# TencentAI4S/HuDiff

Measured on AMD Instinct MI355X. Metric: humanized sequences/sec (full T-step sample) on HuAb348, higher is better.
Workload: dtype f32-equivalent: fp16 hi+lo split, 3 MFMA / product, f32 accumulate; pruned tail + static branch f32

## Files before the change

hudiff_amd/csrc/hd_api.hip:

```cpp
#include "../../include/hudiff_hip.h"
#include "hd_kernels.hip.h"
#include "hd_tail_fused.hip.h"
#include "hd_attn_fused.hip.h"
#include "hd_chain.hip.h"

#include <cmath>
#include <cstdarg>
#include <cstdio>
#include <cstdlib>
#include <cstring>
#include <map>
#include <string>
#include <vector>

using namespace hd;

static thread_local std::string g_err;
static thread_local std::string g_launch_err;

static HdStatus fail(HdStatus st, const char* fmt, ...) {
    char buf[1024];
    va_list ap;
    va_start(ap, fmt);
    vsnprintf(buf, sizeof(buf), fmt, ap);
// ... 69 lines not shown
    {HD_OPT_BIG_MIN_ROWS, "HUDIFF_BIG_ROWS", 8192, 1, OPT_BIG, {}, 0, false},
    {HD_OPT_LNSYNC_LEVEL, "HUDIFF_X3_LNSYNC", 2, 0, 2, {}, 0, false},
    {HD_OPT_TAIL_FORM, "HUDIFF_TAIL", 2, 0, 2, {0, 2}, 2, false},
    {HD_OPT_TAIL_MAX_ROWS, "HUDIFF_TAIL_MAX_B", 64, 0, OPT_BIG, {}, 0, false},
    {HD_OPT_SMALL_GRID, "HUDIFF_X3_SMALL_GRID", 320, 0, OPT_BIG, {}, 0, false},
    {HD_OPT_TINY_GRID, "HUDIFF_X3_TINY_GRID", 150, 0, OPT_BIG, {}, 0, false},
    {HD_OPT_LOADER_WAVES, "HUDIFF_X3_LOADERS", 1, 0, 1, {}, 0, false},
    {HD_OPT_TINY_STAGES, "HUDIFF_X3_TINY_NS", 3, 2, 3, {}, 0, false},
    {HD_OPT_SMALL_STAGES, "HUDIFF_X3_SMALL_NS", 0, 0, 3, {0, 2, 3}, 3, false},
    {HD_OPT_SMALL_STAGES3_MAX_GRID, "HUDIFF_X3_SMALL_NS3_MAX", 256, 0, OPT_BIG, {}, 0, false},
    {HD_OPT_ATTN_QSPLIT_MAX_GRID, "HUDIFF_ATTN_QSPLIT_MAX", 128, 0, OPT_BIG, {}, 0, false},
    {HD_OPT_ATTN_WAVES, "HUDIFF_ATTN_WAVES", 12, 8, 12, {8, 12}, 2, false},
    {HD_OPT_LOOP_GRAPH, "HUDIFF_LOOP_GRAPH", 0, 0, 1, {}, 0, false},
    {HD_OPT_PRUNE_VALUE_VIA_ROWS, "HUDIFF_PRUNE_V", 1, 0, 1, {}, 0, false},
    {HD_OPT_SPLIT_TILE, "HUDIFF_X3_TILE", 0, 0, 512, {0, 128, 256, 512}, 4, false},
    {HD_OPT_GEMM_SMALL_TILES, "HUDIFF_GEMM_SMALL", 1536, 0, OPT_BIG, {}, 0, false},
    {HD_OPT_STORE_NT, "HUDIFF_ST_NT", 0, 0, 1, {}, 0, false},
    {HD_OPT_SPLIT_LAYER_MASK, "HUDIFF_X3_MASK", 3, 0, 3, {}, 0, true},
    {HD_OPT_SPLIT_ATTN, "HUDIFF_X3_ATTN", 1, 0, 1, {}, 0, false},
    {HD_OPT_FUSED_ATTN, "HUDIFF_FUSED_ATTN", 1, 0, 1, {}, 0, false},
    {HD_OPT_FUSED_ATTN_MIN_GRID, "HUDIFF_FUSED_ATTN_MIN_GRID", 128, 0, OPT_BIG, {}, 0, false},
    {HD_OPT_BN_CHAIN, "HUDIFF_BN_CHAIN", 0, 0, 3, {}, 0, true},
    {HD_OPT_BN_CHAIN_MIN_TILES, "HUDIFF_BN_CHAIN_MIN_TILES", 128, 0, OPT_BIG, {}, 0, false},
};
static bool opt_legal(const OptDef& d, int64_t v) {
    if (v < d.lo || v > d.hi) return false;
    if (d.nset == 0) return true;
    for (int i = 0; i < d.nset; ++i) if (d.set[i] == v) return true;
    return false;
}

struct HdModel {
    HdConfig cfg{};
    int device = 0;
    hipStream_t stream = nullptr;
    bool finalized = false;
    std::map<std::string, HostTensor> host;
    int nseg = 1, d = 0, dh = 0, D = 0, Dh = 0, A = 0, Fd = 0, L = 0;
    float p_enc = 0.f, p_conv = 0.f;
    float* blob = nullptr;
    uint16_t* blobx = nullptr;
    int precision_req = HD_PRECISION_DEFAULT, precision = HD_PRECISION_SPLIT;
    int64_t opt[HD_OPT_COUNT] = {};
    bool debug_lnsync_scatter = false;
    bool x3 = false;
    bool x3_suspended = false;
    int64_t range_fallbacks = 0;
    bool attn_x3 = true;
    int lnsync_level_cfg = 2, lnsync_level = 2;
    int64_t lnsync_fallbacks = 0;
    bool last_call_repeated = false;
    bool lnsync_cross_xcd = false;
    const float* emb = nullptr;
    std::vector<ByteNetW> enc, conv;
    std::vector<AttBlockW> att;
    RegionW regw{};
    SideW sidew{};
    const float *pos_w1 = nullptr, *pos_b1 = nullptr, *pos_w2 = nullptr, *pos_b2 = nullptr;
    HeadW head{};
    const float *rope_cos = nullptr, *rope_sin = nullptr, *rope_cs = nullptr;
    float* side_vec = nullptr;
    float2* emb_stats = nullptr;
    float* qnoise = nullptr; size_t qnoise_cap = 0;
    struct Lane {
        hipStream_t stream = nullptr;
        RunState* rs = nullptr;
        Workspace ws;
// ... 83 lines not shown
    if (c.kind != HD_KIND_ANTIBODY && c.kind != HD_KIND_NANOBODY) return fail(HD_ERR_INVALID, "hd_create: kind %d", c.kind);
    if (c.att_model != c.nhead * ATT_HD)
        return fail(HD_ERR_UNSUPPORTED, "hd_create: head dim %d/%d unsupported (kernels implement 64)", c.att_model, c.nhead);
    const int nkt = (c.max_len + 15) / 16;
    if (nkt != 19 && nkt != 10)
        return fail(HD_ERR_UNSUPPORTED, "hd_create: max_len %d unsupported (291 or 152)", c.max_len);
    if (c.d_model % 8 || c.sum_d_model % 8 || c.dim_feedforward % 4 || c.d_model > 512 || c.sum_d_model > 1024)
        return fail(HD_ERR_UNSUPPORTED, "hd_create: widths must be multiples of 8 (d_model<=512, sum_d_model<=1024)");
    if (c.r_embedding > 8 || c.s_embedding > 8 || c.n_tokens < 23 || c.n_tokens > 64)
        return fail(HD_ERR_UNSUPPORTED, "hd_create: r_embedding/s_embedding <= 8, n_tokens in [23,64]");
    if (c.kind == HD_KIND_ANTIBODY) {
        if (c.h_len <= 0 || c.h_len >= c.max_len) return fail(HD_ERR_INVALID, "hd_create: h_len %d", c.h_len);
        if (c.sum_d_model != 3 * c.d_model) return fail(HD_ERR_INVALID, "hd_create: sum_d_model != 3*d_model");
    } else {
        if (c.h_len != c.max_len) return fail(HD_ERR_INVALID, "hd_create: nanobody h_len must equal max_len");
        if (c.sum_d_model != 2 * c.d_model) return fail(HD_ERR_INVALID, "hd_create: sum_d_model != 2*d_model");
    }
    if (c.kernel_size != 7 && c.kernel_size != 5 && c.kernel_size != 3)
        return fail(HD_ERR_UNSUPPORTED, "hd_create: kernel_size %d", c.kernel_size);
    if (!(c.dropout >= 0.f && c.dropout < 1.f)) return fail(HD_ERR_INVALID, "hd_create: dropout %f", c.dropout);
    for (int a : {c.enc_act, c.conv_act})
        if (a != HD_ACT_RELU && a != HD_ACT_GELU) return fail(HD_ERR_INVALID, "hd_create: activation %d", a);

    int ndev = hd_device_count();
    if (ndev <= 0) return fail(HD_ERR_NO_DEVICE, "hd_create: no HIP device visible (this library has no CPU path)");
    if (device < 0 || device >= ndev) return fail(HD_ERR_INVALID, "hd_create: device %d out of range [0,%d)", device, ndev);
    HIP_TRY(hipSetDevice(device));
    hipDeviceProp_t prop;
    HIP_TRY(hipGetDeviceProperties(&prop, device));
    if (strncmp(prop.gcnArchName, "gfx950", 6) != 0)
        return fail(HD_ERR_NO_DEVICE, "hd_create: device %d is %s, kernels are built for gfx950 only", device, prop.gcnArchName);
    HdModel* m = new HdModel();
    m->cfg = c;
    for (const OptDef& d : OPTS) {
        m->opt[d.id] = d.def;
        if (const char* e = getenv(d.env)) {
            const int64_t v = atoll(e);
            if (opt_legal(d, v)) m->opt[d.id] = v;
            else {
                if (d.nset == 0) m->opt[d.id] = v < d.lo ? d.lo : d.hi;
                if (!getenv("HUDIFF_QUIET"))
                    fprintf(stderr, "[hudiff_hip] %s=%s is not a legal value of that option: %s %lld\n", d.env, e,
                            d.nset == 0 ? "clamped to" : "ignored, the default stays", (long long)m->opt[d.id]);
            }
        }
    }
    if (!getenv("HUDIFF_QUIET")) {
        static const char* const removed[] = {"HUDIFF_GEMM_NBUF", "HUDIFF_PFF3_APPLY", "HUDIFF_ENC_FUSED", "HUDIFF_ENC_ABL", "HUDIFF_X3_PERSIST"};
        for (const char* r : removed)
            if (getenv(r)) fprintf(stderr, "[hudiff_hip] %s is set, but this build has no such switch any more: ignored\n", r);
    }
    m->device = device;
    m->nseg = c.kind == HD_KIND_ANTIBODY ? 2 : 1;
    m->d = c.d_model; m->dh = c.d_model / 2; m->D = c.sum_d_model; m->Dh = c.sum_d_model / 2;
    m->A = c.att_model; m->Fd = c.dim_feedforward; m->L = c.max_len;
    m->p_enc = c.dropout;
    m->p_conv = c.dropout > 0.f ? 0.5f : 0.f;
    for (auto& ln : m->lane) {
        hipError_t e = hipStreamCreate(&ln.stream);
        if (e != hipSuccess) { delete m; return fail(HD_ERR_HIP, "hipStreamCreate: %s", hipGetErrorString(e)); }
        hipEventCreate(&ln.ev0);
        hipEventCreate(&ln.ev1);
    }
    *out = m;
    return HD_OK;
}
// ... 771 lines not shown
    return x3_use(m, sg, w.a1.wqkvx) && x3_use(m, sg, w.a1.wox) && x3_use(m, sg, w.a2.wqkvx) && x3_use(m, sg, w.a2.wox) &&
           x3_use(m, sg, w.wf1x) && x3_use(m, sg, w.wf2x) && cur(m).ws.YX && cur(m).ws.ATX;
}
static size_t lds_request(int bytes, int threads) {
    static const bool no_pad = [] { const char* e = getenv("HUDIFF_LDS_NO_PAD"); return e && atoi(e) == 1; }();
    return (size_t)(no_pad ? bytes : lds_safe_request(bytes, threads));
}

static void attention_layer(HdModel* m, const Segs& sg, const AttLayerW& w, const float* x, bool ln,
                            const float* resid, float* out, bool want_out_stats, bool x3 = false,
                            const float* x_split = nullptr, float* out_split = nullptr, bool split_only = false) {
    hipStream_t st = cur(m).stream;
    const int D = m->D, A = m->A;
    GemmP p = base_gemm(m, sg);
    p.A = x; p.lda = D; p.W = w.wqkv; p.bias = w.bqkv; p.C = cur(m).ws.QKV; p.ldc = 3 * A; p.N = 3 * A; p.Kc = D;
    if (ln) { p.ln_fold = 1; use_partials(m, p); }
    const bool fuse19 = m->L > 16 * 18 && m->L <= 16 * 19,
               fuse10 = m->L > 16 * 9 && m->L <= 16 * 10 && m->cfg.nhead % 2 == 0 && lds_fill_ok(QaGeom<10, 2>::smem(m->L), QA_THREADS);
    const long fused_blocks = (long)sg.B * (m->cfg.nhead / (fuse19 ? 1 : 2)) * (m->in_session ? m->nlanes : 1);
    if (x3 && x_split && w.wqkvx.w && m->opt[HD_OPT_FUSED_ATTN] && fused_blocks >= m->opt[HD_OPT_FUSED_ATTN_MIN_GRID] && m->opt[HD_OPT_SPLIT_ATTN] && (fuse19 || fuse10) && D % X3_BK == 0 && A % X3_BN == 0 &&
        (long)sg.rows() * 3 * A * 4 < (1L << 31) && (long)sg.rows() * D * 4 < (1L << 31) &&
        m->cfg.nhead * (fuse19 ? 19 : 10) <= sg.len[0] && 2 * A * 4 >= 4096) {
        QkvAttnP q{};
        q.X = x_split; q.ldx = D; q.x_bytes = (uint32_t)((long)sg.rows() * D * 4);
        q.Wx = w.wqkvx.w; q.acc_scale = w.wqkvx.acc_scale; q.bias = w.bqkv;
        q.ln_fold = p.ln_fold; q.stats = p.stats; q.spart = p.spart; q.spw = p.spw; q.spart_rows = p.spart_rows;
        q.QKV = cur(m).ws.QKV; q.ldq = 3 * A; q.att = A; q.rope_cos = m->rope_cos; q.rope_sin = m->rope_sin; q.rope_cs = m->rope_cs;
        q.O = cur(m).ws.O; q.ldo = A; q.nhead = m->cfg.nhead; q.sg = sg; q.rs = cur(m).rs;
#ifdef HD_PROBES
        static const int qa_abl = [] { const char* e = getenv("HUDIFF_QA_ABL"); return e ? atoi(e) : 0; }();
        q.abl = qa_abl;
#endif
        const int NH = fuse19 ? 1 : 2;
        dim3 fgrid((unsigned)(((sg.B + 7) / 8) * 8 * (m->cfg.nhead / NH)));
        tally(m, fuse19 ? HD_DBG_QKV_ATTN_19 : HD_DBG_QKV_ATTN_10);
        if (fuse19) hipLaunchKernelGGL((qkv_attn_x3_k<19, 1>), fgrid, dim3(QA_THREADS), lds_request(QaGeom<19, 1>::smem(m->L), QA_THREADS), st, q);
        else hipLaunchKernelGGL((qkv_attn_x3_k<10, 2>), fgrid, dim3(QA_THREADS), lds_request(QaGeom<10, 2>::smem(m->L), QA_THREADS), st, q);
        p = base_gemm(m, sg);
        p.A = cur(m).ws.O; p.lda = A; p.W = w.wo; p.bias = w.bo; p.C = out; p.ldc = D; p.N = D; p.Kc = A;
        p.resid = resid; p.ldr = D;
        use_x3(p, w.wox); p.C2 = out_split;
        if (split_only && out_split) { p.C = out_split; p.c_split = 1; p.C2 = nullptr; }
        launch_gemm(m, p, false, false, want_out_stats ? STATS_PARTIALS : STATS_NONE);
        return;
    }
    if (x3) { p.A = x_split; use_x3(p, w.wqkvx); }
    launch_gemm(m, p, false, false);
    const size_t smem = lds_request((int)((size_t)m->L * (ATT_KS + att_vs(m->L > 160 ? 19 : 10)) * sizeof(float)), ATT_THREADS);
    dim3 grid(sg.B * m->cfg.nhead);
    const bool ax_on = m->opt[HD_OPT_SPLIT_ATTN] != 0;
    const bool ax_ok = ((x3 && ax_on) || (m->attn_x3 && !m->x3_suspended && sg.rows() >= m->opt[HD_OPT_BIG_MIN_ROWS])) && (long)sg.rows() * 3 * A * 4 < (1L << 31);
    const RunState* rsp = cur(m).rs;
    const int osp = x3 ? 1 : 0;
    const bool ax_kernel = ax_ok && ((m->L > 16 * 18 && m->L <= 16 * 19) || (m->L > 16 * 9 && m->L <= 16 * 10));
    if (ax_kernel && (long)grid.x <= m->opt[HD_OPT_ATTN_QSPLIT_MAX_GRID]) grid.y = 2;
    const bool ax_w8 = m->opt[HD_OPT_ATTN_WAVES] == 8;
    if (grid.y == 2) tally(m, HD_DBG_ATTN_QSPLIT);
    tally(m, !ax_kernel ? HD_DBG_ATTN_F32 : m->L > 160 ? (ax_w8 ? HD_DBG_ATTN_X3_19_W8 : HD_DBG_ATTN_X3_19_W12) : HD_DBG_ATTN_X3_10);
    if (ax_ok && m->L > 16 * 18 && m->L <= 16 * 19 && !ax_w8)
        hipLaunchKernelGGL((attn_x3_k<19, AX19_THREADS>), grid, dim3(AX19_THREADS), lds_request(AxGeom<19>::SMEM, AX19_THREADS), st, cur(m).ws.QKV, 3 * A, A, m->rope_cos, m->rope_sin, cur(m).ws.O, A, m->cfg.nhead, sg, osp, rsp);
    else if (ax_ok && m->L > 16 * 18 && m->L <= 16 * 19)
        hipLaunchKernelGGL(attn_x3_k<19>, grid, dim3(ATT_THREADS), lds_request(AxGeom<19>::SMEM, ATT_THREADS), st, cur(m).ws.QKV, 3 * A, A, m->rope_cos, m->rope_sin, cur(m).ws.O, A, m->cfg.nhead, sg, osp, rsp);
    else if (ax_ok && m->L > 16 * 9 && m->L <= 16 * 10) {
        hipLaunchKernelGGL(attn_x3_k<10>, grid, dim3(ATT_THREADS), lds_request(2 * 128 * m->L + 2 * AxGeom<10>::VPLANE, ATT_THREADS), st, cur(m).ws.QKV, 3 * A, A, m->rope_cos, m->rope_sin, cur(m).ws.O, A, m->cfg.nhead, sg, osp, rsp);
    } else if (m->L > 160)
        hipLaunchKernelGGL(attn_k<19>, grid, dim3(ATT_THREADS), smem, st, cur(m).ws.QKV, 3 * A, A, m->rope_cos, m->rope_sin, cur(m).ws.O, A, m->cfg.nhead, sg, x3 ? 1 : 0, rsp);
    else
// ... 883 lines not shown
```

hudiff_amd/csrc/hd_attn_fused.hip.h:

```cpp
#pragma once
#include "hd_kernels.hip.h"

namespace hd {

struct QkvAttnP {
    const float* X; int ldx; uint32_t x_bytes;
    const uint16_t* Wx; float acc_scale;
    const float* bias;
    int ln_fold; const float2* stats; const float2* spart; int spw; long spart_rows;
    float* QKV; int ldq; int att;
    const float* rope_cos; const float* rope_sin;
    const float* rope_cs;
    float* O; int ldo;
    int nhead; Segs sg; const RunState* rs;
#ifdef HD_PROBES
    int abl;
#endif
};

constexpr int QA_THREADS = 768, QA_WAVES = 12;

template <int KT, int NH>
struct QaGeom {
    typedef AxGeom<KT> G;
    static constexpr int RT = (16 * KT + 31) / 32;
    static constexpr int ROWS = 32 * RT, COLS = 192 * NH, CT = COLS / 32;
    static constexpr int RG = QA_WAVES / CT;
    static constexpr int TM = RT / RG;
    static constexpr int A_BYTES = ROWS * 128, W_BYTES = COLS * 128, STAGE = A_BYTES + W_BYTES;
    static constexpr int A_PIECES = A_BYTES / 1024, W_PIECES = W_BYTES / 1024;
    static constexpr int A_PER_WAVE = (A_PIECES + QA_WAVES - 1) / QA_WAVES, W_PER_WAVE = W_PIECES / QA_WAVES;
    static constexpr int RSTD_OFF = 2 * STAGE;
    __host__ __device__ static constexpr int planes(int L) { return 2 * (KT <= 10 ? L : G::KROWS) * 128 + 2 * G::VPLANE; }
    static constexpr int BIAS_OFF = RSTD_OFF + ROWS * 4;
    __host__ __device__ static constexpr int smem(int L) {
        const int a = NH * planes(L), b = BIAS_OFF + COLS * 4;
        return a > b ? a : b;
    }
    static_assert(RT % RG == 0 && CT * RG == QA_WAVES && W_PIECES % QA_WAVES == 0 && TM == 5, "tile / wave split");
    static_assert(BIAS_OFF + COLS * 4 <= LDS_PER_CU && NH * (2 * G::KROWS * 128 + 2 * G::VPLANE) <= LDS_PER_CU + (KT <= 10 ? 4096 : 0), "LDS");
};

template <int KT, int NH>
__global__ void __launch_bounds__(QA_THREADS, 3) qkv_attn_x3_k(const QkvAttnP p) {
    typedef QaGeom<KT, NH> Q;
    typedef AxGeom<KT> G;
    constexpr int TM = Q::TM, A_BYTES = Q::A_BYTES, W_BYTES = Q::W_BYTES, STAGE = Q::STAGE;
    constexpr bool EXACT = KT <= 10;
    extern __shared__ __attribute__((aligned(16))) char qas[];
    const int L = p.sg.L;
    const int tid = threadIdx.x, lane = tid & 63, wave = __builtin_amdgcn_readfirstlane(tid >> 6);
    const int HG = p.nhead / NH;
    int b, h0;
    {
        const int bid = blockIdx.x, xcd = bid & 7, slot = bid >> 3;
        b = (slot / HG) * 8 + xcd;
        h0 = (slot % HG) * NH;
        if (b >= p.sg.B) return;
    }
    const int rA0 = p.sg.base[0] + b * p.sg.len[0] - p.sg.off[0];
    const int rA1 = p.sg.nseg > 1 ? p.sg.base[1] + b * p.sg.len[1] - p.sg.off[1] : rA0;
    const int roff1 = p.sg.nseg > 1 ? p.sg.off[1] : 0x7fffffff;
    const int nkt = p.ldx / X3_BK;
    const unsigned long long t_entry = (HD_QABL(p) & 32) ? wall_clock64() : 0ull;
    auto stamp = [&](int k) {
        if ((HD_QABL(p) & 32) && h0 == 0 && lane == 0)
            p.QKV[(long)(rA0 + p.sg.off[0]) * p.ldq + 2 * p.att + wave * 8 + k] = (float)(wall_clock64() - t_entry);
    };
    float* rstd_s = reinterpret_cast<float*>(qas + Q::RSTD_OFF);
    float* bias_s = reinterpret_cast<float*>(qas + Q::BIAS_OFF);
    auto row_rstd = [&]() {
        if (tid < Q::COLS) {
            const int hh_ = tid / 192, part_ = (tid % 192) / 64, within = tid % 64;
            bias_s[tid] = p.bias[part_ * p.att + (h0 + hh_) * ATT_HD + within];
        }
        for (int r = tid; r < Q::ROWS; r += QA_THREADS) {
            float v = 1.f;
            if (p.ln_fold && r < L) {
                const long grow = r + (r >= roff1 ? rA1 : rA0);
                v = p.spart ? merge_row_stat(p.spart, p.spw, p.spart_rows, p.ldx, grow).y : p.stats[grow].y;
            }
            rstd_s[r] = v;
        }
    };

    constexpr uint32_t BUF_OOB = 0x80000000u;
    uint32_t a_vo[Q::A_PER_WAVE], w_vo[Q::W_PER_WAVE];
#pragma unroll
    for (int i = 0; i < Q::A_PER_WAVE; ++i) {
        const int piece = QA_WAVES * i + wave;
        const int r = 8 * piece + (lane >> 3);
        const uint32_t a_in = (uint32_t)(((lane & 7) ^ ((r >> 1) & 7)) << 4);
        const long grow = r + (r >= roff1 ? rA1 : rA0);
        a_vo[i] = (piece < Q::A_PIECES && r < L) ? (uint32_t)(grow * p.ldx * 4) + a_in : BUF_OOB;
    }
#pragma unroll
    for (int i = 0; i < Q::W_PER_WAVE; ++i) {
        const int piece = QA_WAVES * i + wave;
        const int plane = piece / (Q::COLS / 16), rg16 = piece % (Q::COLS / 16);
        const int R = rg16 * 16, hh = R / 192, part = (R % 192) / 64, within = R % 64;
        const int col = part * p.att + (h0 + hh) * ATT_HD + within;
        w_vo[i] = (uint32_t)((col / X3_BN) * nkt * X3_TILE_BYTES + plane * (X3_TILE_BYTES / 2) + (col % X3_BN) * 64 + lane * 16);
    }
    const __amdgpu_buffer_rsrc_t a_rs = __builtin_amdgcn_make_buffer_rsrc(const_cast<float*>(p.X), 0, (int)p.x_bytes, 0x00020000);
    const __amdgpu_buffer_rsrc_t w_rs = __builtin_amdgcn_make_buffer_rsrc(const_cast<uint16_t*>(p.Wx), 0, (3 * p.att / X3_BN) * nkt * X3_TILE_BYTES, 0x00020000);
    typedef __attribute__((address_space(3))) void* lds_vp;
    auto dma = [&](int kt, int st) {
        char* dst = qas + st * STAGE;
#pragma unroll
        for (int i = 0; i < Q::A_PER_WAVE; ++i)
            if (QA_WAVES * i + wave < Q::A_PIECES)
                __builtin_amdgcn_raw_ptr_buffer_load_lds(a_rs, (lds_vp)(dst + (QA_WAVES * i + wave) * 1024), 16, (int)a_vo[i], kt * X3_BK * 4, 0, 0);
#pragma unroll
        for (int i = 0; i < Q::W_PER_WAVE; ++i) {
            const int piece = QA_WAVES * i + wave;
            const int plane = piece / (Q::COLS / 16), rg16 = piece % (Q::COLS / 16);
            __builtin_amdgcn_raw_ptr_buffer_load_lds(w_rs, (lds_vp)(dst + A_BYTES + plane * (W_BYTES / 2) + rg16 * 1024), 16, (int)w_vo[i],
                                                     kt * X3_TILE_BYTES, 0, 0);
        }
    };

    const int ct = wave % Q::CT, rg = wave / Q::CT;
    const int hh = ct / 6, part = (ct % 6) >> 1, half = ct & 1;
    f32x16 acc[TM];
#pragma unroll
    for (int i = 0; i < TM; ++i)
#pragma unroll
        for (int r = 0; r < 16; ++r) acc[i][r] = 0.f;
    const int fsw = (lane >> 2) & 3, fg = lane >> 5, asw = (lane >> 1) & 7;
    const int foff0 = (lane & 31) * 64 + (((0 + fg) ^ fsw) << 4), foff1 = (lane & 31) * 64 + (((2 + fg) ^ fsw) << 4);
    const int aoff0 = (lane & 31) * 128 + (((0 + fg) ^ asw) << 4), aoff1 = (lane & 31) * 128 + (((4 + fg) ^ asw) << 4);
    constexpr int XROW = 128;
    auto load_x = [&](const char* At, int oa, auto i0_c, auto n_c, f16x8* xh, f16x8* xl) {
        constexpr int I0 = decltype(i0_c)::value, N = decltype(n_c)::value;
#pragma unroll
        for (int i = 0; i < N; ++i) {
            xh[i] = *reinterpret_cast<const f16x8*>(At + oa + 32 * XROW * (I0 + i));
            xl[i] = *reinterpret_cast<const f16x8*>(At + (oa ^ 32) + 32 * XROW * (I0 + i));
        }
    };
    auto mm = [&](auto sw_c, auto i0_c, auto n_c, const f16x8* xh, const f16x8* xl, const f16x8 wh, const f16x8 wl) {
        constexpr bool SW = decltype(sw_c)::value;
        constexpr int I0 = decltype(i0_c)::value, N = decltype(n_c)::value;
#pragma unroll
        for (int i = 0; i < N; ++i) acc[I0 + i] = SW ? __builtin_amdgcn_mfma_f32_32x32x16_f16(wh, xl[i], acc[I0 + i], 0, 0, 0)
                                                     : __builtin_amdgcn_mfma_f32_32x32x16_f16(xl[i], wh, acc[I0 + i], 0, 0, 0);
#pragma unroll
        for (int i = 0; i < N; ++i) acc[I0 + i] = SW ? __builtin_amdgcn_mfma_f32_32x32x16_f16(wl, xh[i], acc[I0 + i], 0, 0, 0)
                                                     : __builtin_amdgcn_mfma_f32_32x32x16_f16(xh[i], wl, acc[I0 + i], 0, 0, 0);
#pragma unroll
        for (int i = 0; i < N; ++i) acc[I0 + i] = SW ? __builtin_amdgcn_mfma_f32_32x32x16_f16(wh, xh[i], acc[I0 + i], 0, 0, 0)
                                                     : __builtin_amdgcn_mfma_f32_32x32x16_f16(xh[i], wh, acc[I0 + i], 0, 0, 0);
    };
    constexpr int WAIT_ALL = 0x0F70;
    const int khalf = lane >> 5, l31 = lane & 31;
    const int hcol = (h0 + hh) * ATT_HD;
    const float sc = p.acc_scale;
    const int krows = EXACT ? L : G::KROWS;
    auto wave_program = [&](auto part_c) {
        using std::integral_constant;
        constexpr int PART = decltype(part_c)::value;
        constexpr std::integral_constant<bool, PART != 2> sw_c{};
        constexpr integral_constant<int, 0> c0{}; constexpr integral_constant<int, 2> c2{}; constexpr integral_constant<int, 3> c3{};
        dma(0, 0);
        row_rstd();
        __builtin_amdgcn_s_waitcnt(WAIT_ALL);
        lds_barrier();
#ifdef HD_QA_STAMPS
        uint32_t ts[8] = {0, 0, 0, 0, 0, 0, 0, 0};
#endif
        if (HD_QABL(p) & 1) {
            for (int kt = 0, st = 0; kt < nkt; ++kt, st ^= 1) {
                if (kt + 1 < nkt && !(HD_QABL(p) & 2)) dma(kt + 1, st ^ 1);
                __builtin_amdgcn_s_waitcnt(WAIT_ALL);
                lds_barrier();
            }
        } else {
            f16x8 a0h[3], a0l[3], b0h[2], b0l[2], a1h[3], a1l[3], b1h[2], b1l[2], w0h, w0l, w1h, w1l;
            {
                const char* At = qas + rg * TM * 32 * 128;
                const char* Wt = qas + A_BYTES + ct * 32 * 64;
                w0h = *reinterpret_cast<const f16x8*>(Wt + foff0); w0l = *reinterpret_cast<const f16x8*>(Wt + W_BYTES / 2 + foff0);
                load_x(At, aoff0, c0, c3, a0h, a0l);
            }
            for (int kt = 0, st = 0; kt < nkt; ++kt, st ^= 1) {
#ifdef HD_QA_STAMPS
                if (kt == 10) ts[0] = (uint32_t)__builtin_readcyclecounter();
                if (kt == 11) ts[4] = (uint32_t)__builtin_readcyclecounter();
                if (kt == 12) ts[7] = (uint32_t)__builtin_readcyclecounter();
#endif
                const char* At = qas + st * STAGE + rg * TM * 32 * 128;
                const char* Wt = qas + st * STAGE + A_BYTES + ct * 32 * 64;
                if (kt + 1 < nkt && !(HD_QABL(p) & 2)) dma(kt + 1, st ^ 1);
#ifdef HD_QA_STAMPS
                if (kt == 10) ts[1] = (uint32_t)__builtin_readcyclecounter();
#endif
                load_x(At, aoff0, c3, c2, b0h, b0l);
                __builtin_amdgcn_sched_barrier(0);
// ... 141 lines not shown
                        *reinterpret_cast<f16x4*>(Kl + off) = lv;
                    }
                }
                __builtin_amdgcn_sched_barrier(0);
            }
        } else if constexpr (PART == 2) {
            const int d = 32 * half + l31;
#pragma unroll
            for (int i = 0; i < TM; ++i) {
                const int t = rg * TM + i;
#pragma unroll
                for (int j = 0; j < 4; ++j) {
                    const int o = 8 * j + 4 * khalf;
                    f32x4 x4 = {acc[i][4 * j], acc[i][4 * j + 1], acc[i][4 * j + 2], acc[i][4 * j + 3]};
                    if (32 * t + 32 > L) {
#pragma unroll
                        for (int e = 0; e < 4; ++e) x4[e] = (32 * t + o + e < L) ? x4[e] : 0.f;
                    }
                    f16x4 hv, lv;
                    split4(x4, hv, lv);
                    if (HD_GUARD_MASK & 8) vmax = absmax4(vmax, x4);
                    const int g = (o & 15) >> 2, second = o >> 4;
                    const int off = d * (G::VKEYS * 2) + (G::vpos(4 * t + g, d) << 4) + 8 * second;
                    *reinterpret_cast<f16x4*>(Vh + off) = hv;
                    *reinterpret_cast<f16x4*>(Vl + off) = lv;
                }
            }
        }
        if constexpr (PART != 0) raise_range_flag(p.rs, vmax);
        stamp(3);
        __syncthreads();
        stamp(4);
    };
    if (part == 0) wave_program(std::integral_constant<int, 0>{});
    else if (part == 1) wave_program(std::integral_constant<int, 1>{});
    else wave_program(std::integral_constant<int, 2>{});

    const __amdgpu_buffer_rsrc_t o_rs = __builtin_amdgcn_make_buffer_rsrc(p.O, 0, 0x7fffffff, 0x00020000);
    if (HD_QABL(p) & 4) return;
#pragma unroll
    for (int hx = 0; hx < NH; ++hx) {
        const char* pl = qas + hx * Q::planes(L);
#ifdef HD_QA_STAMPS
        float* cstamps = (h0 == 0 && hx == 0) ? p.QKV + (long)(rA0 + p.sg.off[0] + 2) * p.ldq + 2 * p.att : nullptr;
#else
        float* cstamps = nullptr;
#endif
        attn_x3_tiles<KT, QA_THREADS, true>(pl, pl + krows * 128, pl + 2 * krows * 128, pl + 2 * krows * 128 + G::VPLANE, p.QKV, p.ldq,
                                            (int)((uint32_t)(rA0 + p.sg.off[0] + (h0 + hx) * KT) * (uint32_t)p.ldq * 4u),
                                            p.rope_cos, p.rope_sin, o_rs, p.ldo, b, h0 + hx, p.sg, 1, p.rs, lane, wave, cstamps);
    }
    stamp(5);
}

}
```

hudiff_amd/csrc/hd_kernels.hip.h:

```cpp
#pragma once
#include <hip/hip_runtime.h>
#include <stdint.h>
#include <type_traits>

#if defined(__HIP_DEVICE_COMPILE__) && !defined(__gfx950__)
#error "hd_kernels.hip.h is written for gfx950 (CDNA4) only: wave64, MFMA 32x32x16 f16, buffer_load ... lds, 160 KB LDS, s_barrier semantics of ended waves"
#endif

namespace hd {

typedef float f32x4 __attribute__((ext_vector_type(4)));
typedef float f32x16 __attribute__((ext_vector_type(16)));

#ifdef HD_PROBES
#define HD_ABL(p) ((p).x3_abl)
#define HD_QABL(p) ((p).abl)
#else
#define HD_ABL(p) 0
#define HD_QABL(p) 0
#endif

enum { ACT_NONE = 0, ACT_RELU = 1, ACT_GELU = 2 };
enum { DROP_NONE = 0, DROP_GEN = 1, DROP_INJECT = 2 };
constexpr int PART_STRIDE = 32;
// ... 1489 lines not shown
                f32x4 o = oacc[dt];
                o[0] *= inv; o[1] *= inv; o[2] *= inv; o[3] *= inv;
                const int col = h * ATT_HD + 16 * dt + 4 * g;
                if (o_split) {
                    f16x4 hh, ll;
                    split4(o, hh, ll);
                    if (HD_GUARD_MASK & 4) vmax = absmax4(vmax, o);
                    _Float16* orow = reinterpret_cast<_Float16*>(O + qrow * ldo);
                    const int oc = 128 * h + 4 * g + 32 * dt;
                    *reinterpret_cast<f16x4*>(orow + oc) = hh;
                    *reinterpret_cast<f16x4*>(orow + oc + X16_LO) = ll;
                } else {
                    *reinterpret_cast<f32x4*>(O + qrow * ldo + col) = o;
                }
            }
        }
    }
    if (o_split) raise_range_flag(rs, vmax);
}

template <int KT> struct AxGeom {
    static constexpr int KROWS = 16 * KT, VKEYS = 32 * ((KT + 1) / 2);
    static constexpr int KPLANE = KROWS * 128, VPLANE = 64 * VKEYS * 2;
    static constexpr int SMEM = 2 * KPLANE + 2 * VPLANE;
    static constexpr bool WIDE = (VKEYS * 2) % 256 == 128;
    static_assert(WIDE || (VKEYS * 2) % 256 == 64, "V^T row stride must be 32 or 16 banks modulo 64");
    __device__ static constexpr int vpos(int c, int d) {
        return WIDE ? ((c & ~7) | ((c & 7) ^ ((d >> 1) & 7))) : ((c & ~3) | ((c & 3) ^ ((d >> 2) & 3)));
    }
};
constexpr int AX_KROWS = AxGeom<19>::KROWS;
constexpr int AX19_THREADS = 768;

template <int KT, int NTH, bool QL2>
__device__ __forceinline__ void attn_x3_tiles(const char* Kh, const char* Kl, const char* Vh, const char* Vl, const float* __restrict__ QKV, int ldq,
                                              int qoff, const float* __restrict__ rope_cos, const float* __restrict__ rope_sin,
                                              const __amdgpu_buffer_rsrc_t o_rs, int ldo, int b, int h, const Segs& sg, int o_split,
                                              const RunState* __restrict__ rs, int lane, int wave, float* core_stamps = nullptr) {
    typedef AxGeom<KT> G;
    const unsigned long long cs_t0 = core_stamps ? __builtin_readcyclecounter() : 0ull;
    int cs_tile = 0;
    auto cstamp = [&](int k) {
        if (core_stamps && cs_tile < 2 && lane == 0) core_stamps[wave * 16 + cs_tile * 6 + k] = (float)(__builtin_readcyclecounter() - cs_t0);
    };
    constexpr int AX_KT = KT, AX_VKEYS = G::VKEYS, AX_VPLANE = G::VPLANE;
    constexpr bool EXACT = KT <= 10;
    const int L = sg.L;
    const int qi = lane & 15, g = lane >> 4;
    const int sw = (qi >> 1) & 7;
    const int sw_last = ((L - 1) >> 1) & 7;
    const int nqt = (L + 15) / 16;
    const char* vph[2];
    const char* vpl[2];
#pragma unroll
    for (int par = 0; par < 2; ++par) {
        vph[par] = Vh + qi * (AX_VKEYS * 2) + (G::vpos(4 * par + g, qi) << 4);
        vpl[par] = vph[par] + AX_VPLANE;
    }
    typedef unsigned int u32x4_q __attribute__((ext_vector_type(4)));
    const __amdgpu_buffer_rsrc_t qf_rs = __builtin_amdgcn_make_buffer_rsrc(const_cast<float*>(QKV), 0, 0x7fffffff, 0x00020000);
    f16x8 qh[2], ql[2];
    auto load_qf = [&](int qt) {
        const uint32_t qb = (uint32_t)qoff + (uint32_t)qt * (uint32_t)ldq * 4u + (uint32_t)lane * 16u;
#pragma unroll
        for (int ks = 0; ks < 2; ++ks) {
            qh[ks] = __builtin_bit_cast(f16x8, __builtin_amdgcn_raw_buffer_load_b128(qf_rs, (int)(qb + (uint32_t)(2 * ks) * 1024u), 0, 16));
// ... 42 lines not shown
                const int co1 = ((4 * ks + g) ^ (!EXACT || (kt + 1) * 16 + qi < L ? sw : sw_last)) << 4;
                const f16x8 kh0 = *reinterpret_cast<const f16x8*>(Kh + r0 + co0), kl0 = *reinterpret_cast<const f16x8*>(Kl + r0 + co0);
                f16x8 kh1 = kh0, kl1 = kl0;
                if (two) { kh1 = *reinterpret_cast<const f16x8*>(Kh + r1 + co1); kl1 = *reinterpret_cast<const f16x8*>(Kl + r1 + co1); }
                acc0 = __builtin_amdgcn_mfma_f32_16x16x32_f16(kl0, qh[ks], acc0, 0, 0, 0);
                if (two) acc1 = __builtin_amdgcn_mfma_f32_16x16x32_f16(kl1, qh[ks], acc1, 0, 0, 0);
                acc0 = __builtin_amdgcn_mfma_f32_16x16x32_f16(kh0, ql[ks], acc0, 0, 0, 0);
                if (two) acc1 = __builtin_amdgcn_mfma_f32_16x16x32_f16(kh1, ql[ks], acc1, 0, 0, 0);
                acc0 = __builtin_amdgcn_mfma_f32_16x16x32_f16(kh0, qh[ks], acc0, 0, 0, 0);
                if (two) acc1 = __builtin_amdgcn_mfma_f32_16x16x32_f16(kh1, qh[ks], acc1, 0, 0, 0);
            }
            st[kt] = acc0;
            if (two) st[kt + 1] = acc1;
            __builtin_amdgcn_sched_barrier(0);
        }
        st[AX_KT] = f32x4{0.f, 0.f, 0.f, 0.f};
        if constexpr (QL2) {
            const int qn = qt + (NTH / 64) * (int)gridDim.y;
            if (qn < nqt) load_qf(qn);
        }
        if (core_stamps) { asm volatile("" :: "v"(st[AX_KT - 1])); cstamp(2); }
        float mx = -INFINITY, sum = 0.f;
#pragma unroll
        for (int kt = 0; kt < AX_KT; ++kt)
            {
                if (kt == AX_KT - 1) {
#pragma unroll
                    for (int r = 0; r < 4; ++r)
                        if (kt * 16 + 4 * g + r >= L) st[kt][r] = -INFINITY;
                }
#pragma unroll
                for (int r = 0; r < 4; ++r) mx = fmaxf(mx, st[kt][r]);
            }
        mx = fmaxf(mx, __shfl_xor(mx, 16));
        mx = fmaxf(mx, __shfl_xor(mx, 32));
#pragma unroll
        for (int kt = 0; kt < AX_KT; ++kt)
#pragma unroll
            for (int r = 0; r < 4; ++r) { const float e = __builtin_amdgcn_exp2f(st[kt][r] - mx); st[kt][r] = e; sum += e; }
        sum += __shfl_xor(sum, 16);
        sum += __shfl_xor(sum, 32);
        const float inv = 1.0f / sum;
        if (core_stamps) { asm volatile("" :: "v"(inv)); cstamp(3); }
        f32x4 oacc[4];
#pragma unroll
        for (int dt = 0; dt < 4; ++dt) oacc[dt] = f32x4{0.f, 0.f, 0.f, 0.f};
#pragma unroll
        for (int t = 0; t < (AX_KT + 1) / 2; ++t) {
            f16x8 ph, pl;
#pragma unroll
            for (int q4 = 0; q4 < 2; ++q4) {
                f16x4 h4, l4;
                split4(st[2 * t + q4], h4, l4);
#pragma unroll
                for (int e = 0; e < 4; ++e) { ph[4 * q4 + e] = h4[e]; pl[4 * q4 + e] = l4[e]; }
            }
            if constexpr (KT <= 10 && !QL2) {
#pragma unroll
                for (int dt = 0; dt < 4; ++dt) {
                    const int ro = 128 * (t >> 1) + 16 * dt * (AX_VKEYS * 2);
                    const f16x8 vh = *reinterpret_cast<const f16x8*>(vph[t & 1] + ro), vl = *reinterpret_cast<const f16x8*>(vpl[t & 1] + ro);
                    oacc[dt] = __builtin_amdgcn_mfma_f32_16x16x32_f16(vl, ph, oacc[dt], 0, 0, 0);
                    oacc[dt] = __builtin_amdgcn_mfma_f32_16x16x32_f16(vh, pl, oacc[dt], 0, 0, 0);
                    oacc[dt] = __builtin_amdgcn_mfma_f32_16x16x32_f16(vh, ph, oacc[dt], 0, 0, 0);
                }
            } else
#pragma unroll
            for (int dp = 0; dp < 4; dp += 2) {
                const int ro0 = 128 * (t >> 1) + 16 * dp * (AX_VKEYS * 2), ro1 = ro0 + 16 * (AX_VKEYS * 2);
                const f16x8 vh0 = *reinterpret_cast<const f16x8*>(vph[t & 1] + ro0), vl0 = *reinterpret_cast<const f16x8*>(vpl[t & 1] + ro0);
                const f16x8 vh1 = *reinterpret_cast<const f16x8*>(vph[t & 1] + ro1), vl1 = *reinterpret_cast<const f16x8*>(vpl[t & 1] + ro1);
                oacc[dp] = __builtin_amdgcn_mfma_f32_16x16x32_f16(vl0, ph, oacc[dp], 0, 0, 0);
                oacc[dp + 1] = __builtin_amdgcn_mfma_f32_16x16x32_f16(vl1, ph, oacc[dp + 1], 0, 0, 0);
                oacc[dp] = __builtin_amdgcn_mfma_f32_16x16x32_f16(vh0, pl, oacc[dp], 0, 0, 0);
// ... 458 lines not shown
```

Baseline: 107.4.

## Make fused QKV-attention kernel persistent over a CU-sized grid

The fused QKV+attention kernel now launches at most one block per CU (rounded to a multiple of 8) and each block loops over (batch, head-group) items, striding by the grid size. When the LDS layout allows it (KT>10 with room to hold the planes), the next item's row rstd and bias are prefetched into LDS by waves that would otherwise be idle during the attention tail. The softmax cross-lane reductions also switch from __shfl_xor to a direct ds_bpermute helper. This is meant to cut block-launch and tail overhead and overlap stat loading, at the cost of recomputing per-wave constants each iteration, extra register pressure and possible load imbalance across CUs.

```diff
diff --git a/hudiff_amd/csrc/hd_api.hip b/hudiff_amd/csrc/hd_api.hip
--- a/hudiff_amd/csrc/hd_api.hip
+++ b/hudiff_amd/csrc/hd_api.hip
@@ -125,7 +125,7 @@
 
 struct HdModel {
     HdConfig cfg{};
-    int device = 0;
+    int device = 0, cu_count = 0;
     hipStream_t stream = nullptr;
     bool finalized = false;
     std::map<std::string, HostTensor> host;
@@ -275,6 +275,7 @@
         return fail(HD_ERR_NO_DEVICE, "hd_create: device %d is %s, kernels are built for gfx950 only", device, prop.gcnArchName);
     HdModel* m = new HdModel();
     m->cfg = c;
+    m->cu_count = prop.multiProcessorCount;
     for (const OptDef& d : OPTS) {
         m->opt[d.id] = d.def;
         if (const char* e = getenv(d.env)) {
@@ -1112,7 +1113,13 @@
         q.abl = qa_abl;
 #endif
         const int NH = fuse19 ? 1 : 2;
-        dim3 fgrid((unsigned)(((sg.B + 7) / 8) * 8 * (m->cfg.nhead / NH)));
+        q.items = ((sg.B + 7) / 8) * 8 * (m->cfg.nhead / NH);
+#ifdef HD_QA_ONE_ITEM
+        dim3 fgrid((unsigned)q.items);
+#else
+        const int cu8 = m->cu_count / 8 * 8;
+        dim3 fgrid((unsigned)(cu8 >= 8 && q.items > cu8 ? cu8 : q.items));
+#endif
         tally(m, fuse19 ? HD_DBG_QKV_ATTN_19 : HD_DBG_QKV_ATTN_10);
         if (fuse19) hipLaunchKernelGGL((qkv_attn_x3_k<19, 1>), fgrid, dim3(QA_THREADS), lds_request(QaGeom<19, 1>::smem(m->L), QA_THREADS), st, q);
         else hipLaunchKernelGGL((qkv_attn_x3_k<10, 2>), fgrid, dim3(QA_THREADS), lds_request(QaGeom<10, 2>::smem(m->L), QA_THREADS), st, q);
diff --git a/hudiff_amd/csrc/hd_attn_fused.hip.h b/hudiff_amd/csrc/hd_attn_fused.hip.h
--- a/hudiff_amd/csrc/hd_attn_fused.hip.h
+++ b/hudiff_amd/csrc/hd_attn_fused.hip.h
@@ -13,6 +13,7 @@
     const float* rope_cs;
     float* O; int ldo;
     int nhead; Segs sg; const RunState* rs;
+    int items;
 #ifdef HD_PROBES
     int abl;
 #endif
@@ -30,13 +31,16 @@
     static constexpr int A_BYTES = ROWS * 128, W_BYTES = COLS * 128, STAGE = A_BYTES + W_BYTES;
     static constexpr int A_PIECES = A_BYTES / 1024, W_PIECES = W_BYTES / 1024;
     static constexpr int A_PER_WAVE = (A_PIECES + QA_WAVES - 1) / QA_WAVES, W_PER_WAVE = W_PIECES / QA_WAVES;
-    static constexpr int RSTD_OFF = 2 * STAGE;
     __host__ __device__ static constexpr int planes(int L) { return 2 * (KT <= 10 ? L : G::KROWS) * 128 + 2 * G::VPLANE; }
+    static constexpr int STAT_BYTES = ROWS * 4 + COLS * 4;
+    static constexpr bool HOLD = KT > 10 && lds_fill_ok(NH * (2 * G::KROWS * 128 + 2 * G::VPLANE) + STAT_BYTES, QA_THREADS);
+    static constexpr int RSTD_OFF = HOLD ? NH * (2 * G::KROWS * 128 + 2 * G::VPLANE) : 2 * STAGE;
     static constexpr int BIAS_OFF = RSTD_OFF + ROWS * 4;
     __host__ __device__ static constexpr int smem(int L) {
         const int a = NH * planes(L), b = BIAS_OFF + COLS * 4;
         return a > b ? a : b;
     }
+    static_assert(!HOLD || (RSTD_OFF >= 2 * STAGE && lds_fill_ok(BIAS_OFF + COLS * 4, QA_THREADS)), "rstd / bias above the planes: LDS co-residency rule");
     static_assert(RT % RG == 0 && CT * RG == QA_WAVES && W_PIECES % QA_WAVES == 0 && TM == 5, "tile / wave split");
     static_assert(BIAS_OFF + COLS * 4 <= LDS_PER_CU && NH * (2 * G::KROWS * 128 + 2 * G::VPLANE) <= LDS_PER_CU + (KT <= 10 ? 4096 : 0), "LDS");
 };
@@ -48,18 +52,22 @@
     constexpr int TM = Q::TM, A_BYTES = Q::A_BYTES, W_BYTES = Q::W_BYTES, STAGE = Q::STAGE;
     constexpr bool EXACT = KT <= 10;
     extern __shared__ __attribute__((aligned(16))) char qas[];
-    const int L = p.sg.L;
-    const int tid = threadIdx.x, lane = tid & 63, wave = __builtin_amdgcn_readfirstlane(tid >> 6);
+    int L = p.sg.L;
+    int tid = threadIdx.x, lane = tid & 63, wave = __builtin_amdgcn_readfirstlane(tid >> 6);
     const int HG = p.nhead / NH;
-    int b, h0;
-    {
-        const int bid = blockIdx.x, xcd = bid & 7, slot = bid >> 3;
-        b = (slot / HG) * 8 + xcd;
-        h0 = (slot % HG) * NH;
-        if (b >= p.sg.B) return;
-    }
-    const int rA0 = p.sg.base[0] + b * p.sg.len[0] - p.sg.off[0];
-    const int rA1 = p.sg.nseg > 1 ? p.sg.base[1] + b * p.sg.len[1] - p.sg.off[1] : rA0;
+    int item = blockIdx.x;
+    int b, h0, rA0, rA1;
+    auto item_bh = [&](int it, int& b_, int& h0_) {
+        const int xcd = it & 7, slot = it >> 3;
+        b_ = (slot / HG) * 8 + xcd;
+        h0_ = (slot % HG) * NH;
+    };
+    auto item_rows = [&](int b_, int& r0_, int& r1_) {
+        r0_ = p.sg.base[0] + b_ * p.sg.len[0] - p.sg.off[0];
+        r1_ = p.sg.nseg > 1 ? p.sg.base[1] + b_ * p.sg.len[1] - p.sg.off[1] : r0_;
+    };
+    item_bh(item, b, h0);
+    if (item >= p.items || b >= p.sg.B) return;
     const int roff1 = p.sg.nseg > 1 ? p.sg.off[1] : 0x7fffffff;
     const int nkt = p.ldx / X3_BK;
     const unsigned long long t_entry = (HD_QABL(p) & 32) ? wall_clock64() : 0ull;
@@ -69,16 +77,19 @@
     };
     float* rstd_s = reinterpret_cast<float*>(qas + Q::RSTD_OFF);
     float* bias_s = reinterpret_cast<float*>(qas + Q::BIAS_OFF);
-    auto row_rstd = [&]() {
-        if (tid < Q::COLS) {
-            const int hh_ = tid / 192, part_ = (tid % 192) / 64, within = tid % 64;
-            bias_s[tid] = p.bias[part_ * p.att + (h0 + hh_) * ATT_HD + within];
-        }
-        for (int r = tid; r < Q::ROWS; r += QA_THREADS) {
+    auto row_rstd = [&](int h0_, int r0_, int r1_, int t, auto nt_c) {
+        constexpr int nt = decltype(nt_c)::value;
+        int spw = p.spw, kc = p.ldx;
+        asm volatile("" : "+s"(spw), "+s"(kc));
+        for (int c = t; c < Q::COLS; c += nt) {
+            const int hh_ = c / 192, part_ = (c % 192) / 64, within = c % 64;
+            bias_s[c] = p.bias[part_ * p.att + (h0_ + hh_) * ATT_HD + within];
+        }
+        for (int r = t; r < Q::ROWS; r += nt) {
             float v = 1.f;
             if (p.ln_fold && r < L) {
-                const long grow = r + (r >= roff1 ? rA1 : rA0);
-                v = p.spart ? merge_row_stat(p.spart, p.spw, p.spart_rows, p.ldx, grow).y : p.stats[grow].y;
+                const long grow = r + (r >= roff1 ? r1_ : r0_);
+                v = p.spart ? merge_row_stat(p.spart, spw, p.spart_rows, kc, grow).y : p.stats[grow].y;
             }
             rstd_s[r] = v;
         }
@@ -86,6 +97,8 @@
 
     constexpr uint32_t BUF_OOB = 0x80000000u;
     uint32_t a_vo[Q::A_PER_WAVE], w_vo[Q::W_PER_WAVE];
+    auto item_offsets = [&]() {
+    item_rows(b, rA0, rA1);
 #pragma unroll
     for (int i = 0; i < Q::A_PER_WAVE; ++i) {
         const int piece = QA_WAVES * i + wave;
@@ -102,6 +115,7 @@
         const int col = part * p.att + (h0 + hh) * ATT_HD + within;
         w_vo[i] = (uint32_t)((col / X3_BN) * nkt * X3_TILE_BYTES + plane * (X3_TILE_BYTES / 2) + (col % X3_BN) * 64 + lane * 16);
     }
+    };
     const __amdgpu_buffer_rsrc_t a_rs = __builtin_amdgcn_make_buffer_rsrc(const_cast<float*>(p.X), 0, (int)p.x_bytes, 0x00020000);
     const __amdgpu_buffer_rsrc_t w_rs = __builtin_amdgcn_make_buffer_rsrc(const_cast<uint16_t*>(p.Wx), 0, (3 * p.att / X3_BN) * nkt * X3_TILE_BYTES, 0x00020000);
     typedef __attribute__((address_space(3))) void* lds_vp;
@@ -120,16 +134,22 @@
         }
     };
 
-    const int ct = wave % Q::CT, rg = wave / Q::CT;
-    const int hh = ct / 6, part = (ct % 6) >> 1, half = ct & 1;
+    int ct, rg, hh, part, half;
+    int fsw, fg, asw, foff0, foff1, aoff0, aoff1, khalf, l31;
+    auto wave_consts = [&]() {
+        int t = KT <= 10 ? (int)threadIdx.x : tid, l = p.sg.L;
+        asm volatile("" : "+v"(t));
+        asm volatile("" : "+s"(l));
+        L = l;
+        tid = t; lane = t & 63; wave = __builtin_amdgcn_readfirstlane(t >> 6);
+        ct = wave % Q::CT; rg = wave / Q::CT;
+        hh = ct / 6; part = (ct % 6) >> 1; half = ct & 1;
+        fsw = (lane >> 2) & 3; fg = lane >> 5; asw = (lane >> 1) & 7;
+        foff0 = (lane & 31) * 64 + (((0 + fg) ^ fsw) << 4); foff1 = (lane & 31) * 64 + (((2 + fg) ^ fsw) << 4);
+        aoff0 = (lane & 31) * 128 + (((0 + fg) ^ asw) << 4); aoff1 = (lane & 31) * 128 + (((4 + fg) ^ asw) << 4);
+        khalf = lane >> 5; l31 = lane & 31;
+    };
     f32x16 acc[TM];
-#pragma unroll
-    for (int i = 0; i < TM; ++i)
-#pragma unroll
-        for (int r = 0; r < 16; ++r) acc[i][r] = 0.f;
-    const int fsw = (lane >> 2) & 3, fg = lane >> 5, asw = (lane >> 1) & 7;
-    const int foff0 = (lane & 31) * 64 + (((0 + fg) ^ fsw) << 4), foff1 = (lane & 31) * 64 + (((2 + fg) ^ fsw) << 4);
-    const int aoff0 = (lane & 31) * 128 + (((0 + fg) ^ asw) << 4), aoff1 = (lane & 31) * 128 + (((4 + fg) ^ asw) << 4);
     constexpr int XROW = 128;
     auto load_x = [&](const char* At, int oa, auto i0_c, auto n_c, f16x8* xh, f16x8* xl) {
         constexpr int I0 = decltype(i0_c)::value, N = decltype(n_c)::value;
@@ -153,17 +173,19 @@
                                                      : __builtin_amdgcn_mfma_f32_32x32x16_f16(xh[i], wh, acc[I0 + i], 0, 0, 0);
     };
     constexpr int WAIT_ALL = 0x0F70;
-    const int khalf = lane >> 5, l31 = lane & 31;
-    const int hcol = (h0 + hh) * ATT_HD;
     const float sc = p.acc_scale;
     const int krows = EXACT ? L : G::KROWS;
-    auto wave_program = [&](auto part_c) {
+    auto wave_program = [&](auto part_c, const bool first) {
         using std::integral_constant;
         constexpr int PART = decltype(part_c)::value;
         constexpr std::integral_constant<bool, PART != 2> sw_c{};
         constexpr integral_constant<int, 0> c0{}; constexpr integral_constant<int, 2> c2{}; constexpr integral_constant<int, 3> c3{};
+#pragma unroll
+        for (int i = 0; i < TM; ++i)
+#pragma unroll
+            for (int r = 0; r < 16; ++r) acc[i][r] = 0.f;
         dma(0, 0);
-        row_rstd();
+        if (!Q::HOLD || first) row_rstd(h0, rA0, rA1, tid, std::integral_constant<int, QA_THREADS>{});
         __builtin_amdgcn_s_waitcnt(WAIT_ALL);
         lds_barrier();
 #ifdef HD_QA_STAMPS
@@ -371,12 +393,16 @@
         __syncthreads();
         stamp(4);
     };
-    if (part == 0) wave_program(std::integral_constant<int, 0>{});
-    else if (part == 1) wave_program(std::integral_constant<int, 1>{});
-    else wave_program(std::integral_constant<int, 2>{});
-
     const __amdgpu_buffer_rsrc_t o_rs = __builtin_amdgcn_make_buffer_rsrc(p.O, 0, 0x7fffffff, 0x00020000);
-    if (HD_QABL(p) & 4) return;
+    constexpr int IDLE0 = KT > QA_WAVES && KT < 2 * QA_WAVES ? KT - QA_WAVES : 0;
+    for (bool first = true;; first = false) {
+    wave_consts();
+    item_offsets();
+    if (part == 0) wave_program(std::integral_constant<int, 0>{}, first);
+    else if (part == 1) wave_program(std::integral_constant<int, 1>{}, first);
+    else wave_program(std::integral_constant<int, 2>{}, first);
+
+    if (!(HD_QABL(p) & 4))
 #pragma unroll
     for (int hx = 0; hx < NH; ++hx) {
         const char* pl = qas + hx * Q::planes(L);
@@ -390,6 +416,19 @@
                                             p.rope_cos, p.rope_sin, o_rs, p.ldo, b, h0 + hx, p.sg, 1, p.rs, lane, wave, cstamps);
     }
     stamp(5);
+    item += (int)gridDim.x;
+    if (item >= p.items) break;
+    item_bh(item, b, h0);
+    if (b >= p.sg.B) break;
+    if constexpr (Q::HOLD) {
+        if (wave >= IDLE0) {
+            int r0n, r1n;
+            item_rows(b, r0n, r1n);
+            row_rstd(h0, r0n, r1n, tid - 64 * IDLE0, std::integral_constant<int, 64 * (QA_WAVES - IDLE0)>{});
+        }
+    }
+    lds_barrier();
+    }
 }
 
 }
diff --git a/hudiff_amd/csrc/hd_kernels.hip.h b/hudiff_amd/csrc/hd_kernels.hip.h
--- a/hudiff_amd/csrc/hd_kernels.hip.h
+++ b/hudiff_amd/csrc/hd_kernels.hip.h
@@ -1545,6 +1545,9 @@
 constexpr int AX_KROWS = AxGeom<19>::KROWS;
 constexpr int AX19_THREADS = 768;
 
+__device__ __forceinline__ float lane_xor(float v, int lane, int m) {
+    return __builtin_bit_cast(float, __builtin_amdgcn_ds_bpermute((lane ^ m) << 2, __builtin_bit_cast(int, v)));
+}
 template <int KT, int NTH, bool QL2>
 __device__ __forceinline__ void attn_x3_tiles(const char* Kh, const char* Kl, const char* Vh, const char* Vl, const float* __restrict__ QKV, int ldq,
                                               int qoff, const float* __restrict__ rope_cos, const float* __restrict__ rope_sin,
@@ -1653,14 +1656,14 @@
 #pragma unroll
                 for (int r = 0; r < 4; ++r) mx = fmaxf(mx, st[kt][r]);
             }
-        mx = fmaxf(mx, __shfl_xor(mx, 16));
-        mx = fmaxf(mx, __shfl_xor(mx, 32));
+        mx = fmaxf(mx, lane_xor(mx, lane, 16));
+        mx = fmaxf(mx, lane_xor(mx, lane, 32));
 #pragma unroll
         for (int kt = 0; kt < AX_KT; ++kt)
 #pragma unroll
             for (int r = 0; r < 4; ++r) { const float e = __builtin_amdgcn_exp2f(st[kt][r] - mx); st[kt][r] = e; sum += e; }
-        sum += __shfl_xor(sum, 16);
-        sum += __shfl_xor(sum, 32);
+        sum += lane_xor(sum, lane, 16);
+        sum += lane_xor(sum, lane, 32);
         const float inv = 1.0f / sum;
         if (core_stamps) { asm volatile("" :: "v"(inv)); cstamp(3); }
         f32x4 oacc[4];
```

New measurement: 106.7. About the same (-0.6%).
